# jesselasse/MARL-DMFB

Hardware: AMD Instinct MI355X
Metric: env-steps/sec (whole node), 10x10 DMFB 4-droplet fov9 (higher is better)
Workload: dtype int8 env state/obs + f64 rewards; fp32 Q-net; 1 GPU; DMFB 10x10, drop_num=4, fov=9, 4096 parallel envs per GPU (BASELINE configs[1]); parallelism=dp1: chips sharded per rank, one flat RCCL all-reduce per learn

## Files before the change

marl_dmfb_amd/csrc/crnn_ops.hip:

```cpp
#include <hip/hip_runtime.h>

#include <cstdint>
#include <cstdio>
#include <cstdlib>

#include "../../include/crnn_ops.h"

#define HIP_ABI_TAG "crnn_ops"
#define HIP_ABI_ERR CRNN_ERR_HIP
#include "hip_abi.h"
#include "crnn_mfma.h"
#include "crnn_mfma19.h"
#include "crnn_bwd19.h"

namespace {

constexpr int kBlock = 512;
constexpr int kA1Stride = 52;
constexpr int kDz1Unit = 108;

constexpr int kLdsBudget = 158 * 1024;

template <int OD> struct GeoB {
    static constexpr int DZ2 = 28;
    static constexpr int DZ_ROW = OD * DZ2 + 4;
    static constexpr int ROW_FLOATS = OD * kA1Stride + OD * DZ2 + 4 + 244 + (OD / 2) * kDz1Unit;
    static constexpr int FIXED_FLOATS = OD * OD * 9;
    static constexpr int RBB = ((kLdsBudget / 4 - FIXED_FLOATS) / ROW_FLOATS) < (kBlock / (2 * OD)) ? ((kLdsBudget / 4 - FIXED_FLOATS) / ROW_FLOATS)
                                                                                                   : (kBlock / (2 * OD));
    static constexpr size_t LDS_FLOATS = (size_t)FIXED_FLOATS + (size_t)RBB * ROW_FLOATS + OD * 28;
    static constexpr int UNITS = OD * (OD / 2);
    static constexpr int NA = UNITS >= kBlock ? kBlock : kBlock / 2;
    static constexpr int NB = UNITS - NA;
    static constexpr int XSLICES = NB > 0 ? (kBlock - NA) / NB : 1;
    static_assert(NB >= 0 && (NB == 0 || (NA + NB * XSLICES <= kBlock && XSLICES <= 8)), "dW2 roles");
    static constexpr int ITEMS3 = (OD / 2) * 9;
    static constexpr int RS3 = kBlock / ITEMS3;
    static constexpr int PART = kBlock * 9 + kBlock * 9 + OD + kBlock * 6 + OD;
};

template <int OD>
__global__ __launch_bounds__(kBlock) void k_conv9_bwd(const int8_t *__restrict__ obs, long obs_stride, long rows,
                                                      const float *__restrict__ a2, long a2_stride, const float *__restrict__ g, long g_stride,
                                                      const float *__restrict__ w2, float *__restrict__ part,
                                                      const float *__restrict__ w1, const float *__restrict__ b1) {
    using G = GeoB<OD>;
    extern __shared__ __attribute__((aligned(16))) float lds[];
    float *s_w2 = lds;
    float *s_a1 = s_w2 + OD * OD * 9;
    float *s_dz2 = s_a1 + G::RBB * OD * kA1Stride;
    float *s_in = s_dz2 + G::RBB * G::DZ_ROW;
    float *s_dz1 = s_in + G::RBB * 244;
    float *s_w1 = s_dz1 + G::RBB * (OD / 2) * kDz1Unit;
    const int tid = threadIdx.x;
    for (int i = tid; i < OD * 27; i += kBlock) s_w1[i] = w1[i];
    if (tid < OD) s_w1[OD * 27 + tid] = b1[tid];
    for (int i = tid; i < OD * OD * 9; i += kBlock) {
        const int c2 = i / (OD * 9), rem = i - c2 * OD * 9, c1 = rem / 9, tap = rem - c1 * 9;
        s_w2[(c2 * 9 + tap) * OD + c1] = w2[i];
    }
    float accB2 = 0.0f, accB1 = 0.0f, accB1y = 0.0f;
    float2 accW2[9], accW1[3];
#pragma unroll
    for (int k = 0; k < 9; ++k) accW2[k] = make_float2(0.0f, 0.0f);
#pragma unroll
    for (int k = 0; k < 3; ++k) accW1[k] = make_float2(0.0f, 0.0f);
    const bool pa_full = tid < G::NA;
    const int pa_unit = pa_full ? tid : G::NA + (G::NB > 0 ? (tid - G::NA) % (G::NB > 0 ? G::NB : 1) : 0);
    const int pa_slice = pa_full ? 0 : (G::NB > 0 ? (tid - G::NA) / (G::NB > 0 ? G::NB : 1) : 0);
    const bool pa_on = pa_full || (G::NB > 0 && pa_slice < G::XSLICES);
    const int pa_step = pa_full ? 1 : G::XSLICES;
    const int pa_c2 = pa_unit / (OD / 2), pa_cp = pa_unit - pa_c2 * (OD / 2);
    const int i3 = tid % G::ITEMS3, s3 = tid / G::ITEMS3;
    const bool p3_on = s3 < G::RS3;
    const int cp_3 = i3 / 9, c0_3 = (i3 - cp_3 * 9) / 3, kx_3 = i3 - cp_3 * 9 - c0_3 * 3;

    constexpr int kSplit2 = G::NB > 0 ? 2 : 4, kBase2 = G::NB > 0 ? kBlock / 2 : 0;
    const int q2 = (tid - kBase2) & (kSplit2 - 1), unit2 = tid >= kBase2 ? (tid - kBase2) / kSplit2 : G::RBB * (OD / 2);
    const int r2 = unit2 / (OD / 2), cp2 = unit2 - r2 * (OD / 2);
    const int br = tid / OD, bc = tid - br * OD;

    const long n_blocks = (rows + G::RBB - 1) / G::RBB;
    const long per = (n_blocks + gridDim.x - 1) / gridDim.x;
    const long blk0 = (long)blockIdx.x * per, blk1 = min(n_blocks, blk0 + per);

    typedef float f32x4 __attribute__((ext_vector_type(4)));
    const int lane = tid & 63, wave = tid >> 6, j16 = lane & 15, kq = lane >> 4;
    const int c_nh = (wave >> 1) & 1, c_sub = (wave & 1) + 2 * (wave >> 2), c_ch = c_nh * 16 + j16;
    const bool c_chv = c_ch < OD;
    constexpr int NPD = (G::RBB * OD * 25 + kBlock - 1) / kBlock, NPI = (G::RBB * 243 + kBlock - 1) / kBlock;
    float pfa[NPD], pfg[NPD];
    int pfi[NPI];
#pragma unroll
    for (int u = 0; u < NPD; ++u) { pfa[u] = 0.0f; pfg[u] = 0.0f; }
#pragma unroll
    for (int u = 0; u < NPI; ++u) pfi[u] = 0;
    auto fetch = [&](long b) {
        const long r0 = b * G::RBB;
        const int rvb = b < blk1 ? (int)min((long)G::RBB, rows - r0) : 0;
        if (rvb <= 0) return;
        int t_ = tid;
        asm volatile("" : "+v"(t_));
#pragma unroll
        for (int u = 0; u < NPD; ++u) {
            const int i = min(t_ + u * kBlock, G::RBB * OD * 25 - 1), rr = i / (OD * 25), rem = i - rr * OD * 25;
            const long row = r0 + min(rr, rvb - 1);
            pfa[u] = a2[row * a2_stride + rem];
            pfg[u] = g[row * g_stride + rem];
        }
#pragma unroll
        for (int u = 0; u < NPI; ++u) {
            const int i = min(t_ + u * kBlock, G::RBB * 243 - 1), rr = i / 243, pp = i - rr * 243;
            pfi[u] = obs[(r0 + min(rr, rvb - 1)) * obs_stride + pp];
        }
    };
    fetch(blk0);
    for (long blk = blk0; blk < blk1; ++blk) {
        const long row0 = blk * G::RBB;
        const int rv = (int)min((long)G::RBB, rows - row0);
        __syncthreads();
        int t_ = tid;
        asm volatile("" : "+v"(t_));
#pragma unroll
        for (int u = 0; u < NPD; ++u) {
            const int i = t_ + u * kBlock, rc = i / 25, k = i - rc * 25;
            if (i < G::RBB * OD * 25) s_dz2[(rc / OD) * G::DZ_ROW + (rc % OD) * G::DZ2 + k] = (rc / OD < rv && pfa[u] > 0.0f) ? pfg[u] : 0.0f;
        }
#pragma unroll
        for (int u = 0; u < NPI; ++u) {
            const int i = t_ + u * kBlock, rr = i / 243, pp = i - rr * 243;
            if (i < G::RBB * 243) s_in[rr * 244 + pp] = rr < rv ? (float)pfi[u] : 0.0f;
        }
        __syncthreads();
        int off1[7], goff[3];
        float bw1[7];
        int kq_ = kq, j_ = j16;
        asm volatile("" : "+v"(kq_), "+v"(j_));
#pragma unroll
        for (int s = 0; s < 7; ++s) {
            const int k = 4 * s + kq_, c0 = k / 9, tap = k - c0 * 9;
            off1[s] = k < 27 ? c0 * 81 + (tap / 3) * 9 + tap % 3 : 0;
            const float w = s_w1[(c_chv ? c_ch : 0) * 27 + (k < 27 ? k : 0)];
            bw1[s] = (c_chv && k < 27) ? w : 0.0f;
        }
        const float c_bias = c_chv ? s_w1[OD * 27 + c_ch] : 0.0f;
#pragma unroll
        for (int qt = 0; qt < 3; ++qt) { const int p = qt * 16 + j_; goff[qt] = (p / 7) * 9 + p % 7; }
        for (int rr = c_sub; rr < G::RBB; rr += 4) {
            float cv[3][7];
#pragma unroll
            for (int qt = 0; qt < 3; ++qt)
#pragma unroll
                for (int s = 0; s < 7; ++s) cv[qt][s] = s_in[rr * 244 + goff[qt] + off1[s]];
            f32x4 acc[3];
#pragma unroll
            for (int qt = 0; qt < 3; ++qt) acc[qt] = f32x4{c_bias, c_bias, c_bias, c_bias};
#pragma unroll
            for (int s = 0; s < 7; ++s)
#pragma unroll
                for (int qt = 0; qt < 3; ++qt) acc[qt] = __builtin_amdgcn_mfma_f32_16x16x4f32(cv[qt][s], bw1[s], acc[qt], 0, 0, 0);
            if (c_chv) {
                float *dst = s_a1 + ((rr * (OD / 2) + (c_ch >> 1)) * kA1Stride + kq * 4) * 2 + (c_ch & 1);
#pragma unroll
                for (int qt = 0; qt < 3; ++qt)
#pragma unroll
                    for (int q = 0; q < 4; ++q) dst[(qt * 16 + q) * 2] = fmaxf(acc[qt][q], 0.0f);
            }
        }
        if (c_sub == 0) {
            const int rr = j16 < G::RBB ? j16 : G::RBB - 1;
            f32x4 acc = {c_bias, c_bias, c_bias, c_bias};
#pragma unroll
            for (int s = 0; s < 7; ++s) acc = __builtin_amdgcn_mfma_f32_16x16x4f32(s_in[rr * 244 + 60 + off1[s]], bw1[s], acc, 0, 0, 0);
            if (c_chv) {
#pragma unroll
                for (int q = 0; q < 4; ++q)
                    if (kq * 4 + q < G::RBB) s_a1[(((kq * 4 + q) * (OD / 2) + (c_ch >> 1)) * kA1Stride + 48) * 2 + (c_ch & 1)] = fmaxf(acc[q], 0.0f);
            }
        }
        __syncthreads();
        auto unit_rows = [&](int c2, int cp, int r_begin, int r_step) {
#pragma unroll 1
            for (int rr = r_begin; rr < rv; rr += r_step) {
                float dz[G::DZ2];
                float2 a[kA1Stride];
                const float4 *pd = (const float4 *)__builtin_assume_aligned(s_dz2 + rr * G::DZ_ROW + c2 * G::DZ2, 16);
                const float4 *pa = (const float4 *)__builtin_assume_aligned(s_a1 + (size_t)(rr * (OD / 2) + cp) * 2 * kA1Stride, 16);
#pragma unroll
                for (int j = 0; j < G::DZ2 / 4; ++j) { const float4 t = pd[j]; dz[4 * j] = t.x; dz[4 * j + 1] = t.y; dz[4 * j + 2] = t.z; dz[4 * j + 3] = t.w; }
#pragma unroll
                for (int j = 0; j < kA1Stride / 2; ++j) { const float4 t = pa[j]; a[2 * j] = make_float2(t.x, t.y); a[2 * j + 1] = make_float2(t.z, t.w); }
#pragma unroll
                for (int kx = 0; kx < 3; ++kx)
#pragma unroll
                    for (int ky = 0; ky < 3; ++ky)
#pragma unroll
                        for (int x = 0; x < 5; ++x)
#pragma unroll
                            for (int y = 0; y < 5; ++y) {
                                const float z = dz[x * 5 + y];
                                const float2 v = a[(x + kx) * 7 + y + ky];
                                accW2[kx * 3 + ky].x = fmaf(z, v.x, accW2[kx * 3 + ky].x);
                                accW2[kx * 3 + ky].y = fmaf(z, v.y, accW2[kx * 3 + ky].y);
                            }
            }
        };
        if (tid < G::RBB * OD && br < rv) {
            const float4 *pd = (const float4 *)__builtin_assume_aligned(s_dz2 + br * G::DZ_ROW + bc * G::DZ2, 16);
            float t = 0.0f;
#pragma unroll
            for (int j = 0; j < 6; ++j) { const float4 v = pd[j]; t += (v.x + v.y) + (v.z + v.w); }
            accB2 += t + pd[6].x;
        }
#ifndef CRNN_PROBE_SKIP_P1
        if (pa_on) unit_rows(pa_c2, pa_cp, pa_slice, pa_step);
#endif
#ifndef CRNN_PROBE_SKIP_P2
        const bool p2 = unit2 < G::RBB * (OD / 2) && r2 < rv;
#else
        const bool p2 = false;
#endif
        if (p2) {
            float2 da[49];
#pragma unroll
            for (int k = 0; k < 49; ++k) da[k] = make_float2(0.0f, 0.0f);
            const int cbeg = q2 * (OD / kSplit2), cend = cbeg + OD / kSplit2;
#pragma unroll 1
            for (int c2 = cbeg; c2 < cend; ++c2) {
                float dz[G::DZ2];
                float2 w[9];
                const float4 *pd = (const float4 *)__builtin_assume_aligned(s_dz2 + r2 * G::DZ_ROW + c2 * G::DZ2, 16);
#pragma unroll
                for (int j = 0; j < G::DZ2 / 4; ++j) { const float4 t = pd[j]; dz[4 * j] = t.x; dz[4 * j + 1] = t.y; dz[4 * j + 2] = t.z; dz[4 * j + 3] = t.w; }
#pragma unroll
                for (int k = 0; k < 9; ++k) w[k] = *(const float2 *)(s_w2 + (c2 * 9 + k) * OD + 2 * cp2);
#pragma unroll
                for (int kx = 0; kx < 3; ++kx)
#pragma unroll
                    for (int ky = 0; ky < 3; ++ky)
#pragma unroll
                        for (int x = 0; x < 5; ++x)
#pragma unroll
                            for (int y = 0; y < 5; ++y) {
                                float2 &d = da[(x + kx) * 7 + y + ky];
                                const float z = dz[x * 5 + y];
                                d.x = fmaf(z, w[kx * 3 + ky].x, d.x);
                                d.y = fmaf(z, w[kx * 3 + ky].y, d.y);
                            }
            }
#ifndef CRNN_PROBE_P2_NO_DPP
#pragma unroll
            for (int k = 0; k < 49; ++k) {
                asm volatile("v_add_f32_dpp %0, %0, %0 quad_perm:[1,0,3,2] row_mask:0xf bank_mask:0xf bound_ctrl:1" : "+v"(da[k].x));
                asm volatile("v_add_f32_dpp %0, %0, %0 quad_perm:[1,0,3,2] row_mask:0xf bank_mask:0xf bound_ctrl:1" : "+v"(da[k].y));
            }
            if (kSplit2 == 4) {
                asm volatile("s_nop 1");
#pragma unroll
                for (int k = 0; k < 49; ++k) {
                    asm volatile("v_add_f32_dpp %0, %0, %0 quad_perm:[2,3,0,1] row_mask:0xf bank_mask:0xf bound_ctrl:1" : "+v"(da[k].x));
                    asm volatile("v_add_f32_dpp %0, %0, %0 quad_perm:[2,3,0,1] row_mask:0xf bank_mask:0xf bound_ctrl:1" : "+v"(da[k].y));
                }
            }
#endif
#ifdef CRNN_PROBE_P2_NO_MASK
            if (q2 == 0 && da[0].x == 12345.678f) {
#else
            if (q2 == 0) {
#endif
                const float4 *act = (const float4 *)__builtin_assume_aligned(s_a1 + (size_t)unit2 * 2 * kA1Stride, 16);
                unsigned long long lx = 0, ly = 0;
#pragma unroll
                for (int j = 0; j < 25; ++j) {
                    const float4 a = act[j];
                    lx |= (unsigned long long)((a.x > 0.0f ? 1u : 0u) | (a.z > 0.0f ? 2u : 0u)) << (2 * j);
                    ly |= (unsigned long long)((a.y > 0.0f ? 1u : 0u) | (a.w > 0.0f ? 2u : 0u)) << (2 * j);
                }
                float4 *dst4 = (float4 *)__builtin_assume_aligned(s_dz1 + (size_t)unit2 * kDz1Unit, 16);
                float sx = 0.0f, sy = 0.0f;
#pragma unroll
                for (int j = 0; j < 25; ++j) {
                    float4 o;
                    o.x = (lx >> (2 * j)) & 1 ? da[2 * j].x : 0.0f;
                    o.y = (ly >> (2 * j)) & 1 ? da[2 * j].y : 0.0f;
                    o.z = (2 * j + 1 < 49 && ((lx >> (2 * j + 1)) & 1)) ? da[2 * j + 1 < 49 ? 2 * j + 1 : 0].x : 0.0f;
                    o.w = (2 * j + 1 < 49 && ((ly >> (2 * j + 1)) & 1)) ? da[2 * j + 1 < 49 ? 2 * j + 1 : 0].y : 0.0f;
                    dst4[j] = o;
                    sx += o.x + o.z;
                    sy += o.y + o.w;
                }
                accB1 += sx;
                accB1y += sy;
            }
        }
        __syncthreads();
        fetch(blk + 1);
#ifdef CRNN_PROBE_SKIP_P3
        if (false) {
#else
        if (p3_on) {
#endif
            for (int rr = s3; rr < rv; rr += G::RS3) {
                const float2 *pd = (const float2 *)(s_dz1 + (size_t)(rr * (OD / 2) + cp_3) * kDz1Unit);
                const float *in = s_in + rr * 244 + c0_3 * 81 + kx_3 * 9;
#pragma unroll
                for (int x = 0; x < 7; ++x) {
                    float2 dz[7];
                    float v[9];
#pragma unroll
                    for (int y = 0; y < 7; ++y) dz[y] = pd[x * 7 + y];
#pragma unroll
                    for (int y = 0; y < 9; ++y) v[y] = in[x * 9 + y];
#pragma unroll
                    for (int ky = 0; ky < 3; ++ky)
#pragma unroll
                        for (int y = 0; y < 7; ++y) {
                            typedef float f32x2 __attribute__((ext_vector_type(2)));
                            const f32x2 r = __builtin_elementwise_fma((f32x2){dz[y].x, dz[y].y}, (f32x2){v[y + ky], v[y + ky]},
                                                                      (f32x2){accW1[ky].x, accW1[ky].y});
                            accW1[ky] = make_float2(r.x, r.y);
                        }
                }
            }
        }
    }
    __syncthreads();
    if (tid < G::RBB * OD) s_dz2[OD * 16 + bc * 16 + br] = accB2;
    if (q2 == 0 && unit2 < G::RBB * (OD / 2)) {
        s_dz2[(2 * cp2) * 16 + r2] = accB1;
        s_dz2[(2 * cp2 + 1) * 16 + r2] = accB1y;
    }
    __syncthreads();
    float *pp = part + (size_t)blockIdx.x * G::PART;
#pragma unroll
    for (int k = 0; k < 9; ++k) { pp[tid * 18 + 2 * k] = accW2[k].x; pp[tid * 18 + 2 * k + 1] = accW2[k].y; }
    if (tid < OD) {
        float t = 0.0f;
        for (int k = 0; k < G::RBB; ++k) t += s_dz2[OD * 16 + tid * 16 + k];
        pp[kBlock * 18 + tid] = t;
    }
#pragma unroll
    for (int k = 0; k < 3; ++k) { pp[kBlock * 18 + OD + tid * 6 + k] = accW1[k].x; pp[kBlock * 18 + OD + tid * 6 + 3 + k] = accW1[k].y; }
    if (tid < OD) {
        float t = 0.0f;
        for (int k = 0; k < G::RBB; ++k) t += s_dz2[tid * 16 + k];
        pp[kBlock * 18 + OD + kBlock * 6 + tid] = t;
    }
}

constexpr int kRedY = 16;
template <int OD>
__global__ __launch_bounds__(64 * kRedY) void k_conv9_bwd_reduce(const float *__restrict__ part, int n_part, float *__restrict__ grads) {
    using G = GeoB<OD>;
    __shared__ float s_sum[kRedY][64];
    const int tx = threadIdx.x & 63, ty = threadIdx.x >> 6;
    const int i = blockIdx.x * 64 + tx;
    const int n2 = OD * OD * 9, nb = OD, n1 = OD * 27;
    float acc = 0.0f;
    if (i < n2 + nb + n1 + nb) {
        int off[8], cnt = 0;
        if (i < n2) {
            const int pair = i / 9, tap = i - pair * 9, c2 = pair / OD, c1 = pair - c2 * OD;
            const int unit = c2 * (OD / 2) + (c1 >> 1), comp = 2 * tap + (c1 & 1);
            if (unit < G::NA) off[cnt++] = unit * 18 + comp;
            else
                for (int sl = 0; sl < G::XSLICES && sl < 8; ++sl) off[cnt++] = (G::NA + sl * G::NB + (unit - G::NA)) * 18 + comp;
        } else if (i < n2 + nb) {
            off[cnt++] = kBlock * 18 + (i - n2);
        } else if (i < n2 + nb + n1) {
            const int jx = i - n2 - nb, c1 = jx / 27, r = jx - c1 * 27, ky = r % 3;
            const int item = (c1 >> 1) * 9 + r / 3;
            for (int sl = 0; sl < G::RS3; ++sl) off[cnt++] = kBlock * 18 + OD + (sl * G::ITEMS3 + item) * 6 + (c1 & 1) * 3 + ky;
        } else {
            off[cnt++] = kBlock * 18 + OD + kBlock * 6 + (i - n2 - nb - n1);
        }
        for (int k = 0; k < cnt; ++k) {
            float a0 = 0.0f, a1 = 0.0f;
            int b = ty;
            for (; b + kRedY < n_part; b += 2 * kRedY) { a0 += part[(size_t)b * G::PART + off[k]]; a1 += part[(size_t)(b + kRedY) * G::PART + off[k]]; }
            if (b < n_part) a0 += part[(size_t)b * G::PART + off[k]];
            acc += a0 + a1;
        }
    }
    s_sum[ty][tx] = acc;
    __syncthreads();
    if (ty == 0 && i < n2 + nb + n1 + nb) {
        float t = 0.0f;
#pragma unroll
        for (int k = 0; k < kRedY; ++k) t += s_sum[k][tx];
        grads[i] = t;
    }
}

constexpr int kMlpBlock = 256, kMlpOut = 10, kMlpMaxIn = 18, kMlpMaxParts = 256, kMlpTailLoads = 64;
__device__ unsigned g_mlp_ticket = 0;
__global__ __launch_bounds__(kMlpBlock) void k_mlp_bwd(const int8_t *__restrict__ obs, long obs_stride, int dir_off,
                                                       const int8_t *__restrict__ onehot, int n_actions, long rows,
                                                       const float *__restrict__ x, long x_stride, const float *__restrict__ g, long g_stride,
                                                       int col0, float *part, float *__restrict__ dw, float *__restrict__ db) {
    __shared__ float s_red[kMlpBlock / 64][kMlpOut * (kMlpMaxIn + 1)];
    __shared__ int s_last;
    const int nin = 2 + n_actions, n_part = (int)gridDim.x;
    float acc[kMlpOut][kMlpMaxIn + 1];
#pragma unroll
    for (int o = 0; o < kMlpOut; ++o)
#pragma unroll
        for (int k = 0; k <= kMlpMaxIn; ++k) acc[o][k] = 0.0f;
    for (long r = (long)blockIdx.x * kMlpBlock + threadIdx.x; r < rows; r += (long)gridDim.x * kMlpBlock) {
        float v[kMlpMaxIn];
        v[0] = (float)obs[r * obs_stride + dir_off];
        v[1] = (float)obs[r * obs_stride + dir_off + 1];
#pragma unroll
        for (int k = 0; k < kMlpMaxIn - 2; ++k) v[2 + k] = k < n_actions ? (float)onehot[r * n_actions + k] : 0.0f;
#pragma unroll
        for (int o = 0; o < kMlpOut; ++o) {
            const float gz = x[r * x_stride + col0 + o] > 0.0f ? g[r * g_stride + col0 + o] : 0.0f;
#pragma unroll
            for (int k = 0; k < kMlpMaxIn; ++k)
                if (k < nin) acc[o][k] = fmaf(gz, v[k], acc[o][k]);
            acc[o][kMlpMaxIn] += gz;
        }
    }
    const int lane = threadIdx.x & 63, wave = threadIdx.x >> 6;
#pragma unroll
    for (int o = 0; o < kMlpOut; ++o)
#pragma unroll
        for (int k = 0; k <= kMlpMaxIn; ++k)
            if (k < nin || k == kMlpMaxIn) {
                float t = acc[o][k];
                for (int d = 32; d > 0; d >>= 1) t += __shfl_xor(t, d);
                if (lane == 0) s_red[wave][o * (kMlpMaxIn + 1) + k] = t;
            }
    __syncthreads();
    const int n_out = kMlpOut * (nin + 1);
    for (int i = threadIdx.x; i < n_out; i += kMlpBlock) {
        const int o = i < kMlpOut * nin ? i / nin : i - kMlpOut * nin, k = i < kMlpOut * nin ? i - o * nin : kMlpMaxIn;
        float t = 0.0f;
#pragma unroll
        for (int w = 0; w < kMlpBlock / 64; ++w) t += s_red[w][o * (kMlpMaxIn + 1) + k];
        part[(size_t)i * n_part + blockIdx.x] = t;
    }
    if (!last_workgroup_arrives(&g_mlp_ticket, gridDim.x, &s_last)) return;
    for (int i = threadIdx.x; i < n_out; i += kMlpBlock) {
        const float *p = part + (size_t)i * n_part;
        float t = 0.0f;
        for (int b0 = 0; b0 < n_part; b0 += kMlpTailLoads) {
            float v[kMlpTailLoads];
#pragma unroll
            for (int u = 0; u < kMlpTailLoads; ++u) v[u] = b0 + u < n_part ? partial_load(p + b0 + u) : 0.0f;
#pragma unroll
            for (int u = 0; u < kMlpTailLoads; ++u)
                if (b0 + u < n_part) t += v[u];
        }
        if (i < kMlpOut * nin) dw[i] = t;
        else db[i - kMlpOut * nin] = t;
    }
}

struct LiveRows { const int32_t *chips; const int32_t *n; int rows_per_chip; };

template <int OD, int RBV>
int launch_rb(const int8_t *obs, long obs_stride, long rows, const float *w1, const float *b1, const float *w2, const float *b2,
              float *out, long out_stride, int out_cols, const int8_t *onehot, int n_actions, const float *mlp_w, const float *mlp_b, hipStream_t s,
              LiveRows live = LiveRows{nullptr, nullptr, 1}) {
    using GM = crnn_mfma::GeoM<OD, RBV>;
    const size_t lds = GM::LDS_FLOATS * sizeof(float);
    static LdsLimit lds_limit;
    if (const int rc = lds_limit.raise((const void *)crnn_mfma::k_conv9_mfma<OD, RBV>, lds)) return rc;
    const long n_blocks = (rows + GM::RB - 1) / GM::RB;
    const long resident = 256L * (long)((size_t)160 * 1024 / lds);
    const int grid = (int)(n_blocks < resident ? n_blocks : resident);
    LAUNCH((crnn_mfma::k_conv9_mfma<OD, RBV>), dim3(grid), dim3(crnn_mfma::kBlockM), lds, s, obs, obs_stride, rows, w1, b1, w2, b2,
           out, out_stride, out_cols, onehot, n_actions, mlp_w, mlp_b, live.chips, live.n, live.rows_per_chip);
    return CRNN_OK;
}

template <int OD>
int launch(const int8_t *obs, long obs_stride, long rows, const float *w1, const float *b1, const float *w2, const float *b2,
           float *out, long out_stride, int out_cols, const int8_t *onehot, int n_actions, const float *mlp_w, const float *mlp_b, hipStream_t s,
           LiveRows live = LiveRows{nullptr, nullptr, 1}) {
    return launch_rb<OD, 0>(obs, obs_stride, rows, w1, b1, w2, b2, out, out_stride, out_cols, onehot, n_actions, mlp_w, mlp_b, s, live);
}

template <int OD>
int launch19(const int8_t *obs, long obs_stride, long rows, const float *w1, const float *b1, const float *w3, const float *b3,
             float *out, long out_stride, int out_cols, const int8_t *onehot, int n_actions, const float *mlp_w, const float *mlp_b, hipStream_t s) {
    using GM = crnn_mfma19::Geo<OD>;
    const size_t lds = GM::LDS_FLOATS * sizeof(float);
    static LdsLimit lds_limit;
    if (const int rc = lds_limit.raise((const void *)crnn_mfma19::k_conv19_mfma<OD>, lds)) return rc;
    const long n_blocks = (rows + GM::RB - 1) / GM::RB;
    const int grid = (int)(n_blocks < 256 ? n_blocks : 256);
    LAUNCH((crnn_mfma19::k_conv19_mfma<OD>), dim3(grid), dim3(crnn_mfma19::kBlockM), lds, s, obs, obs_stride, rows, w1, b1, w3,
           b3, out, out_stride, out_cols, onehot, n_actions, mlp_w, mlp_b);
    return CRNN_OK;
}

template <int OD>
int launch_bwd(const int8_t *obs, long obs_stride, long rows, const float *a2, long a2_stride,
               const float *g, long g_stride, const float *w2, float *part, int grid, float *grads, const float *w1, const float *b1,
               hipStream_t s) {
    using G = GeoB<OD>;
    const size_t lds = G::LDS_FLOATS * sizeof(float);
    static LdsLimit lds_limit;
    if (const int rc = lds_limit.raise((const void *)k_conv9_bwd<OD>, lds)) return rc;
    HIP_TRY(launch_status([&] {
        hipLaunchKernelGGL((k_conv9_bwd<OD>), dim3(grid), dim3(kBlock), lds, s, obs, obs_stride, rows, a2, a2_stride, g, g_stride,
                           w2, part, w1, b1);
        const int n_out = OD * OD * 9 + OD + OD * 27 + OD;
        hipLaunchKernelGGL((k_conv9_bwd_reduce<OD>), dim3((n_out + 63) / 64), dim3(64 * kRedY), 0, s, part, grid, grads);
    }));
    return CRNN_OK;
}

template <int OD>
int launch_bwd19(const int8_t *obs, long obs_stride, long rows, const float *a3, long a3_stride, const float *g, long g_stride,
                 const float *w1, const float *b1, const float *w3, const float *b3, float *part, int n_part, float *grads, hipStream_t s) {
    using G = crnn_bwd19::GeoB19<OD>;
    const size_t lds = G::LDS_FLOATS * sizeof(float);
    static LdsLimit lds_limit;
    if (const int rc = lds_limit.raise((const void *)crnn_bwd19::k_conv19_bwd<OD>, lds)) return rc;
    const long n_blocks = (rows + G::RBB - 1) / G::RBB;
    const int grid = (int)(n_blocks < n_part ? n_blocks : n_part);
    HIP_TRY(launch_status([&] {
        hipLaunchKernelGGL((crnn_bwd19::k_conv19_bwd<OD>), dim3(grid), dim3(crnn_bwd19::kBlockB), lds, s, obs, obs_stride, rows, a3, a3_stride, g,
                           g_stride, w1, b1, w3, b3, part);
        hipLaunchKernelGGL((crnn_bwd19::k_conv19_bwd_reduce<OD>), dim3((G::GRADS + 63) / 64), dim3(64 * crnn_bwd19::kRedY19), 0, s, part, grid, grads);
    }));
    return CRNN_OK;
}

}

extern "C" {

int crnn_conv9_forward(const int8_t *d_obs, int64_t obs_stride, int64_t rows, const float *d_w1, const float *d_b1,
                       const float *d_w2, const float *d_b2, int od, float *d_out, int64_t out_stride, void *stream) {
    if (!d_obs || !d_w1 || !d_b1 || !d_w2 || !d_b2 || !d_out || rows < 0 || obs_stride < 243 || out_stride < od * 25)
        return CRNN_ERR_BAD_ARG;
    if (rows == 0) return CRNN_OK;
    if (od == 24) return launch<24>(d_obs, obs_stride, rows, d_w1, d_b1, d_w2, d_b2, d_out, out_stride, 0, nullptr, 0, nullptr, nullptr, (hipStream_t)stream);
    if (od == 32) return launch<32>(d_obs, obs_stride, rows, d_w1, d_b1, d_w2, d_b2, d_out, out_stride, 0, nullptr, 0, nullptr, nullptr, (hipStream_t)stream);
    return CRNN_ERR_UNSUPPORTED;
}

int crnn_front9_forward(const int8_t *d_obs, int64_t obs_stride, const int8_t *d_onehot, int n_actions, int64_t rows,
                        const float *d_w1, const float *d_b1, const float *d_w2, const float *d_b2, const float *d_mlp_w,
                        const float *d_mlp_b, int od, float *d_out, int64_t out_stride, int out_cols, void *stream) {
    if (!d_obs || !d_w1 || !d_b1 || !d_w2 || !d_b2 || !d_mlp_w || !d_mlp_b || !d_out || rows < 0 || obs_stride < 245 ||
        out_stride < od * 25 + 10 || n_actions < 0 || n_actions > 16)
        return CRNN_ERR_BAD_ARG;
    if (od != 24 && od != 32) return CRNN_ERR_UNSUPPORTED;
    if (out_cols != 0 && (out_cols < od * 25 + 10 || out_cols > crnn_front_padded_cols(od) || out_cols > out_stride)) return CRNN_ERR_BAD_ARG;
    if (rows == 0) return CRNN_OK;
    if (od == 24) return launch<24>(d_obs, obs_stride, rows, d_w1, d_b1, d_w2, d_b2, d_out, out_stride, out_cols, d_onehot, n_actions, d_mlp_w, d_mlp_b, (hipStream_t)stream);
    return launch<32>(d_obs, obs_stride, rows, d_w1, d_b1, d_w2, d_b2, d_out, out_stride, out_cols, d_onehot, n_actions, d_mlp_w, d_mlp_b, (hipStream_t)stream);
}

int crnn_front9_forward_live(const int8_t *d_obs, int64_t obs_stride, const int8_t *d_onehot, int n_actions, int64_t rows,
                             const float *d_w1, const float *d_b1, const float *d_w2, const float *d_b2, const float *d_mlp_w,
                             const float *d_mlp_b, int od, float *d_out, int64_t out_stride, int out_cols, const int32_t *d_live_chips,
                             const int32_t *d_n_live, int rows_per_chip, void *stream) {
    if (!d_obs || !d_w1 || !d_b1 || !d_w2 || !d_b2 || !d_mlp_w || !d_mlp_b || !d_out || rows < 0 || obs_stride < 245 ||
        out_stride < od * 25 + 10 || n_actions < 0 || n_actions > 16 || !d_live_chips || !d_n_live || rows_per_chip < 1 ||
        rows_per_chip > 64 || rows % rows_per_chip != 0 || rows >= (1 << 25))
        return CRNN_ERR_BAD_ARG;
    if (od != 24 && od != 32) return CRNN_ERR_UNSUPPORTED;
    if (out_cols != 0 && (out_cols < od * 25 + 10 || out_cols > crnn_front_padded_cols(od) || out_cols > out_stride)) return CRNN_ERR_BAD_ARG;
    if (rows == 0) return CRNN_OK;
    const LiveRows live{d_live_chips, d_n_live, rows_per_chip};
    if (od == 24) return launch<24>(d_obs, obs_stride, rows, d_w1, d_b1, d_w2, d_b2, d_out, out_stride, out_cols, d_onehot, n_actions, d_mlp_w, d_mlp_b, (hipStream_t)stream, live);
    return launch<32>(d_obs, obs_stride, rows, d_w1, d_b1, d_w2, d_b2, d_out, out_stride, out_cols, d_onehot, n_actions, d_mlp_w, d_mlp_b, (hipStream_t)stream, live);
}

int crnn_front_padded_cols(int od) { return od == 24 ? crnn_mfma::GeoM<24>::PAD_COLS : od == 32 ? crnn_mfma::GeoM<32>::PAD_COLS : CRNN_ERR_UNSUPPORTED; }

int crnn_front19_forward(const int8_t *d_obs, int64_t obs_stride, const int8_t *d_onehot, int n_actions, int64_t rows,
                         const float *d_w1, const float *d_b1, const float *d_w3, const float *d_b3, const float *d_mlp_w,
                         const float *d_mlp_b, int od, float *d_out, int64_t out_stride, int out_cols, void *stream) {
    const bool vec = d_mlp_w != nullptr;
    const int n_feat = od * 25 + (vec ? 10 : 0);
    if (!d_obs || !d_w1 || !d_b1 || !d_w3 || !d_b3 || !d_out || rows < 0 || obs_stride < 3 * 19 * 19 + (vec ? 2 : 0) ||
        out_stride < n_feat || n_actions < 0 || n_actions > 16 || (vec && !d_mlp_b))
        return CRNN_ERR_BAD_ARG;
    if (od != 24 && od != 32) return CRNN_ERR_UNSUPPORTED;
    if (out_cols != 0 && (out_cols < n_feat || out_cols > crnn_front_padded_cols(od) || out_cols > out_stride)) return CRNN_ERR_BAD_ARG;
    if (rows == 0) return CRNN_OK;
    if (od == 24) return launch19<24>(d_obs, obs_stride, rows, d_w1, d_b1, d_w3, d_b3, d_out, out_stride, out_cols, d_onehot, n_actions, d_mlp_w, d_mlp_b, (hipStream_t)stream);
    return launch19<32>(d_obs, obs_stride, rows, d_w1, d_b1, d_w3, d_b3, d_out, out_stride, out_cols, d_onehot, n_actions, d_mlp_w, d_mlp_b, (hipStream_t)stream);
}

int crnn_conv9_backward_parts(int od) { return od == 24 ? GeoB<24>::PART : od == 32 ? GeoB<32>::PART : CRNN_ERR_UNSUPPORTED; }

int crnn_conv9_backward(const int8_t *d_obs, int64_t obs_stride, int64_t rows, const float *d_out, int64_t out_stride,
                        const float *d_grad_out, int64_t grad_stride, const float *d_w1, const float *d_b1, const float *d_w2,
                        int od, float *d_part, int n_part, float *d_grads, void *stream) {
    if (!d_obs || !d_out || !d_grad_out || !d_w1 || !d_b1 || !d_w2 || !d_part || !d_grads || rows <= 0 || n_part < 1 || n_part > 256)
        return CRNN_ERR_BAD_ARG;
    if (od == 24) return launch_bwd<24>(d_obs, obs_stride, rows, d_out, out_stride, d_grad_out, grad_stride, d_w2, d_part, n_part, d_grads, d_w1, d_b1, (hipStream_t)stream);
    if (od == 32) return launch_bwd<32>(d_obs, obs_stride, rows, d_out, out_stride, d_grad_out, grad_stride, d_w2, d_part, n_part, d_grads, d_w1, d_b1, (hipStream_t)stream);
    return CRNN_ERR_UNSUPPORTED;
}

int crnn_mlp_backward_parts(void) { return kMlpMaxParts * kMlpOut * (kMlpMaxIn + 1); }

int crnn_mlp_backward(const int8_t *d_obs, int64_t obs_stride, int dir_offset, const int8_t *d_onehot, int n_actions, int64_t rows,
                      const float *d_out, int64_t out_stride, const float *d_grad_out, int64_t grad_stride, int col0, float *d_part,
                      float *d_grad_w, float *d_grad_b, void *stream) {
    if (!d_obs || !d_onehot || !d_out || !d_grad_out || !d_part || !d_grad_w || !d_grad_b || rows <= 0 || n_actions < 0 ||
        n_actions > kMlpMaxIn - 2 || dir_offset < 0 || obs_stride < dir_offset + 2 || col0 < 0 || out_stride < col0 + kMlpOut ||
        grad_stride < col0 + kMlpOut)
        return CRNN_ERR_BAD_ARG;
    const long want = (rows + kMlpBlock - 1) / kMlpBlock;
    const int grid = (int)(want < kMlpMaxParts ? want : kMlpMaxParts);
    LAUNCH(k_mlp_bwd, dim3(grid), dim3(kMlpBlock), 0, (hipStream_t)stream, d_obs, (long)obs_stride, dir_offset, d_onehot, n_actions,
           (long)rows, d_out, (long)out_stride, d_grad_out, (long)grad_stride, col0, d_part, d_grad_w, d_grad_b);
    return CRNN_OK;
}

int crnn_conv19_backward_parts(int od) { return od == 24 ? crnn_bwd19::GeoB19<24>::PART : od == 32 ? crnn_bwd19::GeoB19<32>::PART : CRNN_ERR_UNSUPPORTED; }

int crnn_conv19_backward(const int8_t *d_obs, int64_t obs_stride, int64_t rows, const float *d_out, int64_t out_stride,
                         const float *d_grad_out, int64_t grad_stride, const float *d_w1, const float *d_b1, const float *d_w3,
                         const float *d_b3, int od, float *d_part, int n_part, float *d_grads, void *stream) {
    if (!d_obs || !d_out || !d_grad_out || !d_w1 || !d_b1 || !d_w3 || !d_b3 || !d_part || !d_grads || rows <= 0 || n_part < 1 ||
        n_part > 256 || obs_stride < 3 * 19 * 19 || out_stride < od * 25 || grad_stride < od * 25)
        return CRNN_ERR_BAD_ARG;
    if (od == 24) return launch_bwd19<24>(d_obs, obs_stride, rows, d_out, out_stride, d_grad_out, grad_stride, d_w1, d_b1, d_w3, d_b3, d_part, n_part, d_grads, (hipStream_t)stream);
    if (od == 32) return launch_bwd19<32>(d_obs, obs_stride, rows, d_out, out_stride, d_grad_out, grad_stride, d_w1, d_b1, d_w3, d_b3, d_part, n_part, d_grads, (hipStream_t)stream);
    return CRNN_ERR_UNSUPPORTED;
}

int crnn_last_hip_error(void) { return g_last_hip; }

}
```

Baseline: 7.548 million env-steps/s.

## Wave-chunked coalesced prefetch, pipelined dz1 mask loads, strength-reduced phase-3 LDS offsets

The global prefetch of a2/g/obs in the conv9 backward kernel now gives each wave a row-contiguous 64-element chunk. Chunk indices are wave-uniform (readfirstlane, SGPR), so per-lane division by 25/243 drops out and loads coalesce within a row. The LDS scatter uses a checked multiply-shift for div-25. The dz1 masking no longer builds 64-bit masks: it double-buffers activation float4 loads in groups of five with sched barriers. Phase-3 LDS pointers are now incremental offsets. Register pressure and scheduling may change.

```diff
diff --git a/marl_dmfb_amd/csrc/crnn_ops.hip b/marl_dmfb_amd/csrc/crnn_ops.hip
--- a/marl_dmfb_amd/csrc/crnn_ops.hip
+++ b/marl_dmfb_amd/csrc/crnn_ops.hip
@@ -20,6 +20,12 @@
 constexpr int kDz1Unit = 108;
 
 constexpr int kLdsBudget = 158 * 1024;
+
+constexpr bool div25_exact(int n) {
+    for (int e = 0; e < n; ++e)
+        if ((int)(((unsigned)e * 5243u) >> 17) != e / 25) return false;
+    return true;
+}
 
 template <int OD> struct GeoB {
     static constexpr int DZ2 = 28;
@@ -38,6 +44,8 @@
     static constexpr int RS3 = kBlock / ITEMS3;
     static constexpr int PART = kBlock * 9 + kBlock * 9 + OD + kBlock * 6 + OD;
 };
+
+static_assert(GeoB<24>::RBB == 10 && GeoB<32>::RBB == 6 && GeoB<24>::LDS_FLOATS * 4 <= 160 * 1024 && GeoB<32>::LDS_FLOATS * 4 <= 160 * 1024, "LDS budget");
 
 template <int OD>
 __global__ __launch_bounds__(kBlock) void k_conv9_bwd(const int8_t *__restrict__ obs, long obs_stride, long rows,
@@ -88,7 +96,10 @@
     const int lane = tid & 63, wave = tid >> 6, j16 = lane & 15, kq = lane >> 4;
     const int c_nh = (wave >> 1) & 1, c_sub = (wave & 1) + 2 * (wave >> 2), c_ch = c_nh * 16 + j16;
     const bool c_chv = c_ch < OD;
-    constexpr int NPD = (G::RBB * OD * 25 + kBlock - 1) / kBlock, NPI = (G::RBB * 243 + kBlock - 1) / kBlock;
+    constexpr int CHD = (OD * 25 + 63) / 64, NCHD = G::RBB * CHD, NPD = (NCHD + 7) / 8;
+    constexpr int CHI = 4, NCHI = G::RBB * CHI, NPI = (NCHI + 7) / 8;
+    static_assert(div25_exact(64 * CHD), "position split of the park");
+    const int wave_u = __builtin_amdgcn_readfirstlane(wave);
     float pfa[NPD], pfg[NPD];
     int pfi[NPI];
 #pragma unroll
@@ -99,19 +110,21 @@
         const long r0 = b * G::RBB;
         const int rvb = b < blk1 ? (int)min((long)G::RBB, rows - r0) : 0;
         if (rvb <= 0) return;
-        int t_ = tid;
-        asm volatile("" : "+v"(t_));
+        int w_ = wave_u;
+        asm volatile("" : "+s"(w_));
+        const unsigned lane4 = (unsigned)lane * 4u;
 #pragma unroll
         for (int u = 0; u < NPD; ++u) {
-            const int i = min(t_ + u * kBlock, G::RBB * OD * 25 - 1), rr = i / (OD * 25), rem = i - rr * OD * 25;
+            const int ch = min(w_ + 8 * u, NCHD - 1), rr = ch / CHD, v = ch - rr * CHD;
             const long row = r0 + min(rr, rvb - 1);
-            pfa[u] = a2[row * a2_stride + rem];
-            pfg[u] = g[row * g_stride + rem];
+            const unsigned off = min(lane4, (unsigned)(OD * 25 - 1 - 64 * v) * 4u);
+            pfa[u] = *(const float *)((const char *)(a2 + row * a2_stride + 64 * v) + off);
+            pfg[u] = *(const float *)((const char *)(g + row * g_stride + 64 * v) + off);
         }
 #pragma unroll
         for (int u = 0; u < NPI; ++u) {
-            const int i = min(t_ + u * kBlock, G::RBB * 243 - 1), rr = i / 243, pp = i - rr * 243;
-            pfi[u] = obs[(r0 + min(rr, rvb - 1)) * obs_stride + pp];
+            const int ch = min(w_ + 8 * u, NCHI - 1), rr = ch / CHI, v = ch - rr * CHI;
+            pfi[u] = (obs + (r0 + min(rr, rvb - 1)) * obs_stride + 64 * v)[min((unsigned)lane, (unsigned)(242 - 64 * v))];
         }
     };
     fetch(blk0);
@@ -119,17 +132,20 @@
         const long row0 = blk * G::RBB;
         const int rv = (int)min((long)G::RBB, rows - row0);
         __syncthreads();
-        int t_ = tid;
-        asm volatile("" : "+v"(t_));
-#pragma unroll
-        for (int u = 0; u < NPD; ++u) {
-            const int i = t_ + u * kBlock, rc = i / 25, k = i - rc * 25;
-            if (i < G::RBB * OD * 25) s_dz2[(rc / OD) * G::DZ_ROW + (rc % OD) * G::DZ2 + k] = (rc / OD < rv && pfa[u] > 0.0f) ? pfg[u] : 0.0f;
-        }
-#pragma unroll
-        for (int u = 0; u < NPI; ++u) {
-            const int i = t_ + u * kBlock, rr = i / 243, pp = i - rr * 243;
-            if (i < G::RBB * 243) s_in[rr * 244 + pp] = rr < rv ? (float)pfi[u] : 0.0f;
+        {
+            int w_ = wave_u;
+            asm volatile("" : "+s"(w_));
+#pragma unroll
+            for (int u = 0; u < NPD; ++u) {
+                const int ch = w_ + 8 * u, rr = ch / CHD, v = ch - rr * CHD;
+                const unsigned e = (unsigned)(64 * v) + (unsigned)lane, c = (e * 5243u) >> 17;
+                if (ch < NCHD && e < (unsigned)(OD * 25)) s_dz2[rr * G::DZ_ROW + e + 3u * c] = (rr < rv && pfa[u] > 0.0f) ? pfg[u] : 0.0f;
+            }
+#pragma unroll
+            for (int u = 0; u < NPI; ++u) {
+                const int ch = w_ + 8 * u, rr = ch / CHI, pp = 64 * (ch - rr * CHI) + lane;
+                if (ch < NCHI && pp < 243) s_in[rr * 244 + pp] = rr < rv ? (float)pfi[u] : 0.0f;
+            }
         }
         __syncthreads();
         int off1[7], goff[3];
@@ -269,25 +285,36 @@
             if (q2 == 0) {
 #endif
                 const float4 *act = (const float4 *)__builtin_assume_aligned(s_a1 + (size_t)unit2 * 2 * kA1Stride, 16);
-                unsigned long long lx = 0, ly = 0;
-#pragma unroll
-                for (int j = 0; j < 25; ++j) {
-                    const float4 a = act[j];
-                    lx |= (unsigned long long)((a.x > 0.0f ? 1u : 0u) | (a.z > 0.0f ? 2u : 0u)) << (2 * j);
-                    ly |= (unsigned long long)((a.y > 0.0f ? 1u : 0u) | (a.w > 0.0f ? 2u : 0u)) << (2 * j);
-                }
                 float4 *dst4 = (float4 *)__builtin_assume_aligned(s_dz1 + (size_t)unit2 * kDz1Unit, 16);
                 float sx = 0.0f, sy = 0.0f;
-#pragma unroll
-                for (int j = 0; j < 25; ++j) {
-                    float4 o;
-                    o.x = (lx >> (2 * j)) & 1 ? da[2 * j].x : 0.0f;
-                    o.y = (ly >> (2 * j)) & 1 ? da[2 * j].y : 0.0f;
-                    o.z = (2 * j + 1 < 49 && ((lx >> (2 * j + 1)) & 1)) ? da[2 * j + 1 < 49 ? 2 * j + 1 : 0].x : 0.0f;
-                    o.w = (2 * j + 1 < 49 && ((ly >> (2 * j + 1)) & 1)) ? da[2 * j + 1 < 49 ? 2 * j + 1 : 0].y : 0.0f;
-                    dst4[j] = o;
-                    sx += o.x + o.z;
-                    sy += o.y + o.w;
+                float4 an[5];
+#pragma unroll
+                for (int t = 0; t < 5; ++t) an[t] = act[t];
+#pragma unroll
+                for (int jb = 0; jb < 25; jb += 5) {
+                    float4 ac[5];
+#pragma unroll
+                    for (int t = 0; t < 5; ++t) ac[t] = an[t];
+                    if (jb + 5 < 25) {
+#pragma unroll
+                        for (int t = 0; t < 5; ++t) an[t] = act[jb + 5 + t];
+                    }
+                    __builtin_amdgcn_sched_barrier(0);
+#pragma unroll
+                    for (int t = 0; t < 5; ++t) {
+                        const int j = jb + t;
+                        const float4 a = ac[t];
+                        const bool mx = a.x > 0.0f, my = a.y > 0.0f, mz = a.z > 0.0f, mw = a.w > 0.0f;
+                        float4 o;
+                        o.x = mx ? da[2 * j].x : 0.0f;
+                        o.y = my ? da[2 * j].y : 0.0f;
+                        o.z = (2 * j + 1 < 49 && mz) ? da[2 * j + 1 < 49 ? 2 * j + 1 : 0].x : 0.0f;
+                        o.w = (2 * j + 1 < 49 && mw) ? da[2 * j + 1 < 49 ? 2 * j + 1 : 0].y : 0.0f;
+                        dst4[j] = o;
+                        sx += o.x + o.z;
+                        sy += o.y + o.w;
+                    }
+                    __builtin_amdgcn_sched_barrier(0);
                 }
                 accB1 += sx;
                 accB1y += sy;
@@ -300,9 +327,12 @@
 #else
         if (p3_on) {
 #endif
-            for (int rr = s3; rr < rv; rr += G::RS3) {
-                const float2 *pd = (const float2 *)(s_dz1 + (size_t)(rr * (OD / 2) + cp_3) * kDz1Unit);
-                const float *in = s_in + rr * 244 + c0_3 * 81 + kx_3 * 9;
+            static_assert((OD * OD * 9 + G::RBB * (OD * kA1Stride + G::DZ_ROW + 244)) % 4 == 0 && kDz1Unit % 4 == 0, "dz1 units are 16-byte aligned");
+            int o_d = ((int)(s_dz1 - lds) + (s3 * (OD / 2) + cp_3) * kDz1Unit) / 4, o_i = (int)(s_in - lds) + s3 * 244 + c0_3 * 81 + kx_3 * 9;
+            asm volatile("" : "+v"(o_d), "+v"(o_i));
+            for (int rr = s3; rr < rv; rr += G::RS3, o_d += G::RS3 * (OD / 2) * kDz1Unit / 4, o_i += G::RS3 * 244) {
+                const float2 *pd = (const float2 *)((const float4 *)lds + o_d);
+                const float *in = lds + o_i;
 #pragma unroll
                 for (int x = 0; x < 7; ++x) {
                     float2 dz[7];
```

Result: no change. 7.572 million env-steps/s (median of 2 runs) (+0.3%).
